# google-deepmind/bsuite

Hardware: NVIDIA H100
Metric: env-steps/sec (higher is better)
Workload: dtype u32 lane state, f64 reward, f32 observation

## Files before the change

bsuite_b200/csrc/bsb_dispatch.cuh:

```cuda
#pragma once
#include <type_traits>
#include <vector>

#include "bsb_env.h"

namespace bsb {

template <class F> struct HostEmit {
  template <class R> static void run(const EnvParams& p, const typename F::Lane& L, R&, float* dst) { F::row(p, L, dst, 1); }
};
template <> struct HostEmit<UmbrellaChain> {
  template <class R> static void run(const EnvParams& p, const UmbrellaChain::Lane& L, R& r, float* dst) { UmbrellaChain::row(p, L, r, dst, 1); }
};
template <> struct HostEmit<DeepSea> {
  template <class R> static void run(const EnvParams& p, const DeepSea::Lane& L, R&, float* dst) {
    for (int e = 0; e < p.obs_numel; ++e) dst[e] = 0.f;
    if (L.hot >= 0) dst[L.hot] = 1.f;
  }
};
template <> struct HostEmit<Catch> {
  template <class R> static void run(const EnvParams& p, const Catch::Lane& L, R&, float* dst) {
    for (int e = 0; e < p.obs_numel; ++e) dst[e] = 0.f;
    dst[L.hot_a] = 1.f; dst[L.hot_b] = 1.f;
  }
};
template <> struct HostEmit<Mnist> {
  template <class R> static void run(const EnvParams& p, const Mnist::Lane& L, R&, float* dst) {
    if (L.image < 0) { for (int e = 0; e < p.obs_numel; ++e) dst[e] = 0.f; return; }
    const int8_t* src = p.images + (int64_t)L.image * p.obs_numel;
    for (int e = 0; e < p.obs_numel; ++e) dst[e] = Mnist::pixel(src[e]);
  }
};

template <class F, int RK, class O, bool kSameStep = false, bool kPacked = false>
void host_run(const EnvParams& p, const LaunchArgs& a) {
  typedef typename RngOf<RK>::type R;
  const int64_t B = p.batch;
  const int K = p.obs_numel;
  O* const obs = reinterpret_cast<O*>(a.obs);
  O* const fin = reinterpret_cast<O*>(a.final_obs);
  std::vector<float> f32(std::is_same<O, float>::value ? 0 : (size_t)K);
  const bool noise = p.wrapper == BSB_WRAP_REWARD_NOISE && a.mode != MODE_INIT;
  const bool track = p.ep != nullptr && a.mode != MODE_INIT;
  const MailFields out = {a.reward, a.reward_f64, a.discount, a.step_type};
  EnvParams setting_p;
  auto render = [&](const EnvParams& lp, const typename F::Lane& L, R& rng, O* dst) {
    if constexpr (std::is_same<O, float>::value) {
      HostEmit<F>::run(lp, L, rng, dst);
    } else {
      HostEmit<F>::run(lp, L, rng, f32.data());
      for (int e = 0; e < K; ++e) dst[e] = obs_cast<O>(f32[(size_t)e]);
    }
  };
  for (int64_t lane = 0; lane < B; ++lane) {
    if constexpr (kPacked) { setting_p = p; pack_lane_params(setting_p, lane); }
    const EnvParams& lp = kPacked ? setting_p : p;
    typename F::Lane L;
    R rng, wrng;
    EpisodeStats ep;
    ActionStream action_stream;
    action_stream.open();
    lane_open<F>(lp, lane, L, rng, wrng, ep, a.mode, noise, track);
    if (a.mode == MODE_INIT) F::ctor_draws(lp, L, rng);
    MergedReset<F, R> merged;
    F::init(p, merged.last);
    merged.done = false;
    for (int64_t t = 0; t < a.T; ++t) {
      const int64_t off = t * B + lane;
      int32_t action = 0;
      if (a.mode == MODE_STEP) {
        action = a.actions ? a.actions[off]
                           : action_stream.sample(a.action_seed, lp.lane_offset + (uint64_t)lane, (uint64_t)(a.step0 + t), p.num_actions);
        if (a.actions_out) a.actions_out[off] = action;
      }
      lane_step<F, R, kSameStep>(lp, lane, L, rng, wrng, ep, action, a.mode, noise, track, a.step0 + t, out, off, &merged);
      if constexpr (kSameStep) { if (merged.done && fin) render(lp, merged.last, merged.rng, fin + off * (int64_t)K); }
      render(lp, L, rng, obs + off * (int64_t)K);
    }
    lane_close<F>(lp, lane, L, rng, wrng, ep, noise, track);
  }
}

struct Geometry { int threads = 0; size_t smem = 0; int64_t n_chunks = 0, grid = 0; int extra_blocks = 0; };

template <class F, class O>
int plan_launch(bsb_env* e, LaunchArgs& a, Geometry& g, bool no_obs = false, int extra_threads = 0) {
  const int K = e->p.obs_numel;
  const bool is_onehot = EmitKind<F>::value == EMIT_ONEHOT;
  const bool is_image = EmitKind<F>::value == EMIT_IMAGE;
  const int64_t B = e->p.batch;
  a.emit_bulk = 1;
  a.group_lanes = 1;
  a.work_counter = nullptr;
  a.work_base = 0;
  const size_t elem = sizeof(O);
  a.stage_rows = ((size_t)2 * 32 * (size_t)K * elem <= 14 * 1024) ? 2 : 1;
  if (a.T == 1 && (EmitKind<F>::value == EMIT_ROWS || EmitKind<F>::value == EMIT_TWOHOT)) a.stage_rows = 1;
  a.cta_extra_elems = 0;
  a.bad_action = e->bad_action_dev;
  int chunk = 32;
  if (is_image)
    while (chunk > 8 && (B + chunk - 1) / chunk < 4 * (int64_t)e->num_sms) chunk >>= 1;
  a.chunk_lanes = chunk;
  g.n_chunks = (B + chunk - 1) / chunk;
  int threads = 64;
  bool persistent = false;
  const size_t tile = (size_t)K * elem;
  if (is_onehot && a.emit_bulk && g.n_chunks >= 4 * (int64_t)e->num_sms && in_compressed_block(a.obs)) a.emit_bulk = 0;
  if (is_onehot && a.emit_bulk) {
    int m = 1;
    while (m < 16 && (size_t)(2 * m) * tile <= 40 * 1024) m <<= 1;
    if (((size_t)m * tile) % 16 != 0 || (size_t)TILE_STAGES * m * tile > 100 * 1024) {
      a.emit_bulk = 0;
    } else {
      a.group_lanes = m; threads = 32; persistent = true;
    }
  }
  if (is_image && a.emit_bulk) {
    int m = 4;
    while (m > 1 && (size_t)m * tile > 28 * 1024) m >>= 1;
    int mz = 8;
    while (mz > 1 && (size_t)mz * tile > 28 * 1024) mz >>= 1;
    if ((K & 15) != 0 || (size_t)m * tile > 64 * 1024) {
      a.emit_bulk = 0;
    } else {
      a.group_lanes = m; a.stage_rows = 1; threads = 128; a.cta_extra_elems = mz * K; persistent = true;
      if (g.n_chunks < 2 * (int64_t)e->num_sms) threads = 64;
    }
  }
  a.use_pdl = (a.mode == MODE_STEP && a.T == 1) ? 1 : 0;
  if (no_obs) { a.emit_bulk = 0; a.stage_rows = 0; a.cta_extra_elems = 0; a.group_lanes = 1; threads = 128; persistent = false; }
  size_t per_warp = smem_elems_per_warp<F, O>(K, a.emit_bulk != 0, a.group_lanes, a.stage_rows) * elem;
  if ((EmitKind<F>::value == EMIT_ROWS || EmitKind<F>::value == EMIT_TWOHOT) && per_warp > 96 * 1024) {
    a.emit_bulk = 0; a.stage_rows = 0; per_warp = 0;
  }
  const size_t cta_extra = (size_t)a.cta_extra_elems * elem;
  size_t smem = per_warp * (size_t)(threads / 32) + cta_extra;
  while (smem > 96 * 1024 && threads > 32) { threads >>= 1; smem = per_warp * (size_t)(threads / 32) + cta_extra; }
  if (smem > 200 * 1024) return fail(BSB_UNSUPPORTED, "observation too large for the staged emitter");
  g.threads = threads;
  g.smem = smem;
  g.extra_blocks = extra_threads > 0 ? (extra_threads / threads > 1 ? extra_threads / threads : 1) : 0;
  g.grid = (g.n_chunks + threads / 32 - 1) / (threads / 32) + g.extra_blocks;
  if (persistent) {
    int64_t per_sm = (int64_t)((227 * 1024) / (smem + 1024));
    per_sm = per_sm < 1 ? 1 : (per_sm > 16 ? 16 : per_sm);
    const int64_t resident = (int64_t)e->num_sms * per_sm;
    if (g.grid > resident) {
      g.grid = resident;
      a.work_counter = a.clock ? a.clock + CLOCK_CHUNK : e->work_counter;
      a.work_base = a.clock ? 0ull : e->work_base;
    }
  }
  return BSB_OK;
}

template <class Kernel, class... Args>
int launch(bsb_env* e, const LaunchArgs& a, const Geometry& g, cudaStream_t stream, Kernel kernel, const Args&... args) {
  if (g.smem > 48 * 1024) BSB_CUDA(cudaFuncSetAttribute(kernel, cudaFuncAttributeMaxDynamicSharedMemorySize, (int)g.smem));
  cudaLaunchConfig_t cfg;
  memset(&cfg, 0, sizeof(cfg));
  cfg.gridDim = dim3((unsigned)g.grid);
  cfg.blockDim = dim3((unsigned)g.threads);
  cfg.dynamicSmemBytes = g.smem;
  cfg.stream = stream;
  cudaLaunchAttribute attr[1];
  if (a.use_pdl) {
    attr[0].id = cudaLaunchAttributeProgrammaticStreamSerialization;
    attr[0].val.programmaticStreamSerializationAllowed = 1;
    cfg.attrs = attr;
    cfg.numAttrs = 1;
  }
  BSB_CUDA(cudaLaunchKernelEx(&cfg, kernel, args...));
  if (a.work_counter && !a.clock) e->work_base += (unsigned long long)g.n_chunks + (unsigned long long)(g.extra_blocks * (g.threads / 32));
  g_launches.fetch_add(1, std::memory_order_relaxed);
  return BSB_OK;
}

template <class F, int RK, bool kNoise, bool kTrack, class O, bool kSameStep = false>
int device_launch(bsb_env* e, LaunchArgs a, cudaStream_t stream) {
  Geometry g;
  const int rc = plan_launch<F, O>(e, a, g);
  return rc != BSB_OK ? rc : launch(e, a, g, stream, transition_kernel<typename KernelTag<F, O, kSameStep>::type, RK, kNoise, kTrack>, e->p, a);
}

template <class F, int RK, bool kNoise, bool kTrack, class O>
int two_phase_launch(bsb_env* e, LaunchArgs a, TwoPhaseArgs h, cudaStream_t stream) {
  if (a.clock) return fail(BSB_INTERNAL, "a host step reached graph-safe mode, which turns the mailbox path off");
  Geometry g;
  const bool obs_only = h.phase == 2;
  const int rc = plan_launch<F, O>(e, a, g, h.phase == 1, obs_only ? 0 : 512);
  if (rc != BSB_OK) return rc;
  h.copiers = g.extra_blocks;
  return launch(e, a, g, stream, two_phase_host_kernel<typename KernelFamily<F, O>::type, RK, kNoise, kTrack>, e->p, a, h);
}

template <class Launch>
int with_flags(const bsb_env* e, const LaunchArgs& a, Launch launch) {
  const bool noise = e->p.wrapper == BSB_WRAP_REWARD_NOISE && a.mode != MODE_INIT;
  const bool track = e->p.ep != nullptr && a.mode != MODE_INIT;
  if (noise) return track ? launch(std::true_type(), std::true_type()) : launch(std::true_type(), std::false_type());
  return track ? launch(std::false_type(), std::true_type()) : launch(std::false_type(), std::false_type());
}

template <class F, class O, bool kSameStep = false>
int run_family_as(bsb_env* e, const LaunchArgs& a, cudaStream_t stream, const TwoPhaseArgs* two_phase) {
  constexpr bool kF32 = std::is_same<O, float>::value && !kSameStep;
  const bool mt = e->p.rng_kind == BSB_RNG_MT19937;
  if (!kF32 && mt) return fail(BSB_INTERNAL, "reduced obs_dtype or same-step auto-reset with MT19937");
  if (kSameStep && two_phase) return fail(BSB_INTERNAL, "a two-phase host step on a same-step handle");
  if (e->device < 0) {
    if constexpr (kF32) { if (mt) { host_run<F, 1, O>(e->p, a); return BSB_OK; } }
    host_run<F, 0, O, kSameStep>(e->p, a);
    return BSB_OK;
  }
// ... 74 lines not shown
```

bsuite_b200/csrc/bsb_kernels.cuh:

```cuda
#pragma once
#include "bsb_families.cuh"

namespace bsb {

struct MailFields {
  float* reward; double* reward_f64; float* discount; int32_t* step_type;
};

struct LaunchArgs {
  const int32_t* actions;
  int32_t* actions_out;
  float* obs;
  float* reward;
  double* reward_f64;
  float* discount;
  int32_t* step_type;
  int64_t T;
  int64_t step0;
  uint64_t action_seed;
  int32_t mode;
  int32_t obs_vec_ok;
  int32_t emit_bulk;
  int32_t use_pdl;
  int32_t group_lanes;
  int32_t final_vec_ok;
  unsigned long long* work_counter;
  unsigned long long work_base;
  unsigned long long* clock;
  int32_t chunk_lanes;
  int32_t stage_rows;
  int32_t cta_extra_elems;
  struct HostMailbox* mailbox;
  struct DeviceMail* mail;
  unsigned long long ticket;
  int32_t timing;
  float* final_obs;
  int32_t* bad_action;
};

struct TwoPhaseArgs {
  int32_t copiers;
  int32_t phase;
  MailFields stage;
};

struct HostMailbox {
  volatile unsigned long long done;     unsigned long long pad[7];
  volatile unsigned long long stamp[8];
};
struct DeviceMail {
  unsigned long long last_exit;
  unsigned long long finished;
  volatile unsigned long long phase1;
  unsigned long long copied;
};

enum { MODE_STEP = 0, MODE_RESET = 1, MODE_INIT = 2 };

template <class Family, class O> struct ObsAs {};
template <class F> struct FamilyOf { typedef F type; };
template <class Family, class O> struct FamilyOf<ObsAs<Family, O> > { typedef Family type; };
template <class F> struct ObsElemOf { typedef float type; };
template <class Family, class O> struct ObsElemOf<ObsAs<Family, O> > { typedef O type; };
template <class Family, class O> struct KernelFamily { typedef ObsAs<Family, O> type; };
template <class Family> struct KernelFamily<Family, float> { typedef Family type; };
template <class O> struct Vec16 { static const int shift = sizeof(O) == 4 ? 2 : sizeof(O) == 2 ? 3 : 4; };
template <class Family, class O> struct SameStep {};
template <class Family, class O> struct FamilyOf<SameStep<Family, O> > { typedef Family type; };
template <class Family, class O> struct ObsElemOf<SameStep<Family, O> > { typedef O type; };
template <class F> struct IsSameStep { static const bool value = false; };
template <class Family, class O> struct IsSameStep<SameStep<Family, O> > { static const bool value = true; };
template <class Family, class O, bool kSameStep> struct KernelTag { typedef typename KernelFamily<Family, O>::type type; };
template <class Family, class O> struct KernelTag<Family, O, true> { typedef SameStep<Family, O> type; };
template <class Family> struct Packed {};
template <class Family> struct FamilyOf<Packed<Family> > { typedef Family type; };
template <class F> struct IsPacked { static const bool value = false; };
template <class Family> struct IsPacked<Packed<Family> > { static const bool value = true; };

template <int RK> struct RngOf;
template <> struct RngOf<0> { typedef LegacyRng<PhiloxSrc> type; };
template <> struct RngOf<1> { typedef LegacyRng<MtSrc> type; };

BSB_HD void rng_open(LegacyRng<PhiloxSrc>& r, const EnvParams& p, int64_t i, bool wrapper) {
  const uint64_t packed = wrapper ? p.wrng_pos[i] : p.rng_pos[i];
  r.src.open(p.seed, p.lane_offset + (uint64_t)i, wrapper ? STREAM_WRAPPER : STREAM_ENV, packed);
  r.g.has = (packed & RNG_HASGAUSS) ? 1 : 0;
  const double* gz = wrapper ? p.wrng_gauss : p.rng_gauss;
  r.g.value = (r.g.has && gz) ? gz[i] : 0.0;
}
BSB_HD void rng_close(const LegacyRng<PhiloxSrc>& r, const EnvParams& p, int64_t i, bool wrapper) {
  const uint64_t packed = r.src.packed() | (r.g.has ? RNG_HASGAUSS : 0ull);
  if (wrapper) p.wrng_pos[i] = packed; else p.rng_pos[i] = packed;
  double* gz = wrapper ? p.wrng_gauss : p.rng_gauss;
  if (gz && r.g.has) gz[i] = r.g.value;
}
BSB_HD void rng_open(LegacyRng<MtSrc>& r, const EnvParams& p, int64_t i, bool wrapper) {
  const int64_t stride = (p.batch > 0) ? p.batch : 1;
  r.src.open((wrapper ? p.wmt_key : p.mt_key) + i, stride, (wrapper ? p.wmt_idx : p.mt_idx)[i]);
  const uint64_t packed = wrapper ? p.wrng_pos[i] : p.rng_pos[i];
  r.g.has = (packed & RNG_HASGAUSS) ? 1 : 0;
  const double* gz = wrapper ? p.wrng_gauss : p.rng_gauss;
  r.g.value = (r.g.has && gz) ? gz[i] : 0.0;
}
BSB_HD void rng_close(const LegacyRng<MtSrc>& r, const EnvParams& p, int64_t i, bool wrapper) {
  (wrapper ? p.wmt_idx : p.mt_idx)[i] = r.src.idx;
// ... 15 lines not shown
    L.nr = (o.step_type == LAST) ? 1u : 0u;
    if (noise) { o.reward = o.reward + p.noise_scale * wrng.randn(); }
    else if (p.wrapper == 2) { o.reward = o.reward * p.reward_scale; }
  }
  return o;
}

template <class F, class R>
BSB_HD void lane_open(const EnvParams& p, int64_t lane, typename F::Lane& L, R& rng, R& wrng, EpisodeStats& ep,
                      int32_t mode, bool noise, bool track, bool state_loaded = false) {
  if (!state_loaded) { if (mode == MODE_INIT) F::init(p, L); else F::load(p, lane, L); }
  if (p.rng_pos) rng_open(rng, p, lane, false);
  if (noise) rng_open(wrng, p, lane, true);
  if (track && !state_loaded) ep.load(p, lane);
}
template <class F, class R>
BSB_HD void lane_close(const EnvParams& p, int64_t lane, const typename F::Lane& L, const R& rng, const R& wrng,
                       const EpisodeStats& ep, bool noise, bool track) {
  F::store(p, lane, L);
  if (p.rng_pos) rng_close(rng, p, lane, false);
  if (noise) rng_close(wrng, p, lane, true);
  if (track) ep.store(p, lane);
}
template <class F> struct ObsDraws { template <class R> static BSB_HD void skip(const EnvParams&, R&) {} };
template <> struct ObsDraws<UmbrellaChain> {
  template <class R> static BSB_HD void skip(const EnvParams& p, R& rng) {
    for (int k0 = 0; k0 < p.n_distractor; k0 += 64) rng.binomial_half_bits((p.n_distractor - k0) < 64 ? (p.n_distractor - k0) : 64);
  }
};
template <class F, class R> struct MergedReset {
  typename F::Lane last;
  R rng;
  bool done;
};

template <class F, class R, bool kSameStep = false>
BSB_HD void lane_step(const EnvParams& p, int64_t lane, typename F::Lane& L, R& rng, R& wrng, EpisodeStats& ep,
                      int32_t action, int32_t mode, bool noise, bool track, int64_t step, const MailFields& out,
                      int64_t off, MergedReset<F, R>* merged = nullptr) {
  bool after_last = L.nr != 0;
  const StepOut o = lane_transition<F, R, R>(p, lane, L, rng, wrng, action, mode, noise);
  if (track) {
    if constexpr (kSameStep) {
      double* restart = p.ep + 5 * p.batch + lane;
      if (*restart != 0.0) {
        *restart = 0.0;
        if (o.step_type == FIRST) after_last = true;
        else { ep.episode_return = 0.0; p.ep[4 * p.batch + lane] = (double)(step - 1); }
      }
    }
    ep.track(p, lane, o, step, after_last);
    if (p.log_rows && o.step_type == LAST && log_row_due(p, lane)) {
      F::store(p, lane, L); ep.store(p, lane);
      log_row_write(p, lane, step + 1);
    }
  }
  if (out.reward) out.reward[off] = (float)o.reward;
  if (out.reward_f64) out.reward_f64[off] = o.reward;
  if (out.discount) out.discount[off] = o.discount;
  if (out.step_type) out.step_type[off] = o.step_type;
  if constexpr (kSameStep) {
    merged->done = o.step_type == LAST;
    if (merged->done) {
      merged->last = L;
      merged->rng = rng;
      ObsDraws<F>::skip(p, rng);
      F::reset(p, lane, L, rng);
      L.nr = 0;
      if (track) p.ep[5 * p.batch + lane] = 1.0;
    }
  }
}

static const int EMIT_ROWS = 0, EMIT_ONEHOT = 1, EMIT_TWOHOT = 2, EMIT_IMAGE = 3;
template <class F> struct ObsFromState { static const bool value = false; };
template <> struct ObsFromState<DeepSea> { static const bool value = true; };
template <> struct ObsFromState<Catch> { static const bool value = true; };
template <class F> struct EmitKind { static const int value = EMIT_ROWS; };
template <> struct EmitKind<DeepSea> { static const int value = EMIT_ONEHOT; };
template <> struct EmitKind<Catch> { static const int value = EMIT_TWOHOT; };
template <> struct EmitKind<Mnist> { static const int value = EMIT_IMAGE; };
static const int ROW_STAGES = 2;
static const int TILE_STAGES = 2;

template <class F> struct BinaryObs {
  static const bool value = EmitKind<F>::value == EMIT_ONEHOT || EmitKind<F>::value == EMIT_TWOHOT;
};

template <class F, class O> inline
#if defined(__CUDACC__)
__host__ __device__
#endif
size_t smem_elems_per_warp(int K, bool emit_bulk, int group_lanes, int row_stages) {
  if (EmitKind<F>::value == EMIT_ROWS || EmitKind<F>::value == EMIT_TWOHOT) return (size_t)row_stages * 32 * (size_t)K;
  if (EmitKind<F>::value == EMIT_ONEHOT && emit_bulk) return (size_t)TILE_STAGES * (size_t)group_lanes * (size_t)K;
  if (EmitKind<F>::value == EMIT_IMAGE)
    return 256 * sizeof(float) / sizeof(O) + (emit_bulk ? (size_t)group_lanes * (size_t)K : 0);
  return 0;
}

#if defined(__CUDACC__)

__device__ __forceinline__ void st_stream(float4* dst, float4 v) { __stcs(dst, v); }
__device__ __forceinline__ void st_stream(float* dst, float v) { __stcs(dst, v); }
__device__ __forceinline__ void st_stream(Bf16* dst, Bf16 v) { __stcs(reinterpret_cast<unsigned short*>(dst), v.bits); }
__device__ __forceinline__ void st_stream(uint8_t* dst, uint8_t v) { __stcs(dst, v); }
template <class O> __device__ __forceinline__ uint32_t one_bits() {
  return sizeof(O) == 2 ? 0x3f80u : 1u;
}
template <class O> struct Quad;
template <> struct Quad<float> { typedef float4 type; static __device__ __forceinline__ float4 of(float4 v) { return v; } };
template <> struct Quad<Bf16> {
  typedef uint2 type;
  static __device__ __forceinline__ uint2 of(float4 v) {
    return make_uint2((uint32_t)f32_to_bf16_bits(v.x) | ((uint32_t)f32_to_bf16_bits(v.y) << 16),
                      (uint32_t)f32_to_bf16_bits(v.z) | ((uint32_t)f32_to_bf16_bits(v.w) << 16));
  }
};
template <> struct Quad<uint8_t> {
  typedef unsigned int type;
  static __device__ __forceinline__ unsigned int of(float4 v) {
    return (uint32_t)f32_to_u8(v.x) | ((uint32_t)f32_to_u8(v.y) << 8) | ((uint32_t)f32_to_u8(v.z) << 16) |
           ((uint32_t)f32_to_u8(v.w) << 24);
  }
};
__device__ __forceinline__ void st_stream(uint2* dst, uint2 v) { __stcs(dst, v); }
__device__ __forceinline__ void st_stream(unsigned int* dst, unsigned int v) { __stcs(dst, v); }

__device__ __forceinline__ void bulk_store_s2g_hint(void* gdst, const void* ssrc, uint32_t bytes, uint64_t policy) {
  const uint32_t s = (uint32_t)__cvta_generic_to_shared(ssrc);
  asm volatile("cp.async.bulk.global.shared::cta.bulk_group.L2::cache_hint [%0], [%1], %2, %3;" ::"l"(gdst), "r"(s), "r"(bytes), "l"(policy) : "memory");
}
__device__ __forceinline__ uint64_t l2_policy_evict_first() {
  uint64_t p; asm("createpolicy.fractional.L2::evict_first.b64 %0, 1.0;" : "=l"(p)); return p;
}
__device__ __forceinline__ void bulk_store_obs(void* gdst, const void* ssrc, uint32_t bytes) {
  bulk_store_s2g_hint(gdst, ssrc, bytes, l2_policy_evict_first());
}
__device__ __forceinline__ void bulk_commit() { asm volatile("cp.async.bulk.commit_group;" ::: "memory"); }
template <int N> __device__ __forceinline__ void bulk_wait_read() { asm volatile("cp.async.bulk.wait_group.read %0;" ::"n"(N) : "memory"); }
__device__ __forceinline__ void fence_proxy_async_smem() { asm volatile("fence.proxy.async.shared::cta;" ::: "memory"); }
__device__ __forceinline__ void pdl_launch_dependents() { asm volatile("griddepcontrol.launch_dependents;" ::: "memory"); }
__device__ __forceinline__ void pdl_wait() { asm volatile("griddepcontrol.wait;" ::: "memory"); }

template <class O>
__device__ __forceinline__ void emit_onehot_vec(O* obs_t, int64_t warp_base, int n_lanes, int K, int hot, bool vec) {
  const int tid = threadIdx.x & 31;
  if (vec && sizeof(O) != 4) {
    constexpr int S = Vec16<O>::shift;
    const int KV = K >> S;
    for (int j = 0; j < n_lanes; ++j) {
      const int h = __shfl_sync(0xffffffffu, hot, j);
      const int hq = h < 0 ? -1 : (h >> S), hb = (h & ((1 << S) - 1)) * (int)sizeof(O);
      const int word = hb >> 2;
      const uint32_t bits = one_bits<O>() << ((hb & 3) * 8);
      uint4* dst = reinterpret_cast<uint4*>(obs_t + (warp_base + j) * (int64_t)K);
#pragma unroll 8
      for (int q = tid; q < KV; q += 32) {
        uint4 v = make_uint4(0u, 0u, 0u, 0u);
        if (q == hq) { if (word == 0) v.x = bits; else if (word == 1) v.y = bits; else if (word == 2) v.z = bits; else v.w = bits; }
        __stcs(dst + q, v);
      }
    }
  } else if (vec) {
    const int K4 = K >> 2;
    for (int j = 0; j < n_lanes; ++j) {
      const int h = __shfl_sync(0xffffffffu, hot, j);
      const int hq = h >> 2, hc = h & 3;
      float4* dst = reinterpret_cast<float4*>(obs_t + (warp_base + j) * (int64_t)K);
#pragma unroll 8
      for (int q = tid; q < K4; q += 32) {
        float4 v = make_float4(0.f, 0.f, 0.f, 0.f);
        if (q == hq) { if (hc == 0) v.x = 1.f; else if (hc == 1) v.y = 1.f; else if (hc == 2) v.z = 1.f; else v.w = 1.f; }
        st_stream(dst + q, v);
      }
    }
  } else {
    for (int j = 0; j < n_lanes; ++j) {
      const int h = __shfl_sync(0xffffffffu, hot, j);
      O* dst = obs_t + (warp_base + j) * (int64_t)K;
      for (int e = tid; e < K; e += 32) st_stream(dst + e, obs_cast<O>(e == h ? 1.f : 0.f));
    }
  }
}

template <class O>
__device__ __forceinline__ void emit_twohot_vec(O* obs_t, int64_t warp_base, int n_lanes, int K, int hot_a, int hot_b, bool vec) {
  const int tid = threadIdx.x & 31;
  const int total = n_lanes * K;
  O* dst = obs_t + warp_base * (int64_t)K;
  constexpr int S = Vec16<O>::shift;
  if (vec && sizeof(O) != 4 && (total & ((1 << S) - 1)) == 0) {
    const int totalV = total >> S;
    for (int q0 = 0; q0 < totalV; q0 += 32) {
      const int q = q0 + tid;
      const int e0 = (q < totalV ? q : 0) << S;
      int j = e0 / K, c = e0 - j * K;
      uint32_t w[4] = {0u, 0u, 0u, 0u};
#pragma unroll
      for (int k = 0; k < (1 << S); ++k) {
        const int jj = j < 32 ? j : 31;
        const int a = __shfl_sync(0xffffffffu, hot_a, jj);
        const int b = __shfl_sync(0xffffffffu, hot_b, jj);
        if (c == a || c == b) w[(k * (int)sizeof(O)) >> 2] |= one_bits<O>() << (((k * (int)sizeof(O)) & 3) * 8);
        if (++c >= K) { c = 0; ++j; }
      }
      if (q < totalV) __stcs(reinterpret_cast<uint4*>(dst) + q, make_uint4(w[0], w[1], w[2], w[3]));
    }
  } else if (vec && (total & ((1 << S) - 1)) == 0) {
    const int total4 = total >> 2;
    for (int q0 = 0; q0 < total4; q0 += 32) {
      const int q = q0 + tid;
      const int e0 = (q < total4 ? q : 0) << 2;
      int j = e0 / K, c = e0 - j * K;
      float v[4];
#pragma unroll
      for (int k = 0; k < 4; ++k) {
        const int jj = j < 32 ? j : 31;
        const int a = __shfl_sync(0xffffffffu, hot_a, jj);
        const int b = __shfl_sync(0xffffffffu, hot_b, jj);
        v[k] = (c == a || c == b) ? 1.f : 0.f;
        if (++c >= K) { c = 0; ++j; }
      }
      if (q < total4) st_stream(reinterpret_cast<float4*>(dst) + q, make_float4(v[0], v[1], v[2], v[3]));
    }
  } else {
    for (int e0 = 0; e0 < total; e0 += 32) {
      const int e = e0 + tid;
      const int ee = e < total ? e : 0;
      const int j = ee / K, c = ee - j * K;
      const int a = __shfl_sync(0xffffffffu, hot_a, j);
      const int b = __shfl_sync(0xffffffffu, hot_b, j);
      if (e < total) st_stream(dst + e, obs_cast<O>((c == a || c == b) ? 1.f : 0.f));
    }
  }
}

template <class O>
__device__ __forceinline__ void emit_image(const EnvParams& p, const float* lut, O* obs_t, int64_t warp_base, int n_lanes, int K, int image, bool vec) {
  const int tid = threadIdx.x & 31;
  constexpr int U = 8;
  for (int j = 0; j < n_lanes; ++j) {
    const int img = __shfl_sync(0xffffffffu, image, j);
    O* dst = obs_t + (warp_base + j) * (int64_t)K;
    const int8_t* src = p.images + (int64_t)(img < 0 ? 0 : img) * K;
    if (vec) {
      const int K4 = K >> 2;
      const uchar4* src4 = reinterpret_cast<const uchar4*>(src);
      typename Quad<O>::type* dst4 = reinterpret_cast<typename Quad<O>::type*>(dst);
      if (img < 0) {
        for (int q = tid; q < K4; q += 32) st_stream(dst4 + q, Quad<O>::of(make_float4(0.f, 0.f, 0.f, 0.f)));
        continue;
      }
      for (int q0 = 0; q0 < K4; q0 += 32 * U) {
        uchar4 c[U];
#pragma unroll
        for (int u = 0; u < U; ++u) {
          const int q = q0 + u * 32 + tid;
          c[u] = make_uchar4(0, 0, 0, 0);
          if (q < K4) c[u] = __ldg(src4 + q);
        }
#pragma unroll
        for (int u = 0; u < U; ++u) {
          const int q = q0 + u * 32 + tid;
          if (q < K4) st_stream(dst4 + q, Quad<O>::of(make_float4(lut[c[u].x], lut[c[u].y], lut[c[u].z], lut[c[u].w])));
        }
      }
    } else {
// ... 65 lines not shown
          }
      }
      fence_proxy_async_smem();
      __syncwarp();
      if (tid == 0) { bulk_store_obs(dst, buf, bytes); bulk_commit(); }
    }
  }
}

template <class O>
__device__ __forceinline__ void flush_rows_vec(const O* stage, O* obs_t, int64_t warp_base, int n_lanes, int K, bool vec) {
  const int tid = threadIdx.x & 31;
  const int total = n_lanes * K;
  O* dst = obs_t + warp_base * (int64_t)K;
  constexpr int S = Vec16<O>::shift;
  if (vec && (total & ((1 << S) - 1)) == 0) {
    const float4* s4 = reinterpret_cast<const float4*>(stage);
    for (int q = tid; q < (total >> S); q += 32) st_stream(reinterpret_cast<float4*>(dst) + q, s4[q]);
  } else {
    for (int e = tid; e < total; e += 32) st_stream(dst + e, stage[e]);
  }
}

template <class F, class R> struct RowRenderer {
  template <class O> static __device__ __forceinline__ void run(const EnvParams& p, const typename F::Lane& L, R&, O* dst) { F::row(p, L, dst, 1); }
};
template <class R> struct RowRenderer<UmbrellaChain, R> {
  template <class O> static __device__ __forceinline__ void run(const EnvParams& p, const UmbrellaChain::Lane& L, R& r, O* dst) { UmbrellaChain::row(p, L, r, dst, 1); }
};
template <class R> struct RowRenderer<DeepSea, R> { template <class O> static __device__ __forceinline__ void run(const EnvParams&, const DeepSea::Lane&, R&, O*) {} };
template <class R> struct RowRenderer<Catch, R> { template <class O> static __device__ __forceinline__ void run(const EnvParams&, const Catch::Lane&, R&, O*) {} };
template <class R> struct RowRenderer<Mnist, R> { template <class O> static __device__ __forceinline__ void run(const EnvParams&, const Mnist::Lane&, R&, O*) {} };

template <class F> struct Descriptor {
  static __device__ __forceinline__ int a(const typename F::Lane&) { return -1; }
  static __device__ __forceinline__ int b(const typename F::Lane&) { return -1; }
};
template <> struct Descriptor<DeepSea> {
  static __device__ __forceinline__ int a(const DeepSea::Lane& L) { return L.hot; }
  static __device__ __forceinline__ int b(const DeepSea::Lane&) { return -1; }
};
template <> struct Descriptor<Catch> {
  static __device__ __forceinline__ int a(const Catch::Lane& L) { return L.hot_a; }
  static __device__ __forceinline__ int b(const Catch::Lane& L) { return L.hot_b; }
};
template <> struct Descriptor<Mnist> {
  static __device__ __forceinline__ int a(const Mnist::Lane& L) { return L.image; }
  static __device__ __forceinline__ int b(const Mnist::Lane&) { return -1; }
};

template <class F> struct MinBlocksPerSM { static const int value = 4; };
template <> struct MinBlocksPerSM<MemoryChain> { static const int value = 6; };
template <> struct MinBlocksPerSM<Bandit> { static const int value = 8; };
template <> struct MinBlocksPerSM<DiscountingChain> { static const int value = 8; };
#define BSB_LAUNCH_MIN_BLOCKS(F) MinBlocksPerSM<typename FamilyOf<F>::type>::value
__device__ __forceinline__ void st_sys_u64(volatile unsigned long long* ptr, unsigned long long v) {
  asm volatile("st.relaxed.sys.global.u64 [%0], %1;" ::"l"(ptr), "l"(v) : "memory");
}
__device__ __forceinline__ unsigned long long global_timer_ns() {
  unsigned long long t; asm volatile("mov.u64 %0, %%globaltimer;" : "=l"(t)); return t;
}
__device__ __forceinline__ void bulk_wait_all() { asm volatile("cp.async.bulk.wait_group 0;" ::: "memory"); }

static const int CLOCK_GROUPS = 32, CLOCK_CHUNK = 16 * CLOCK_GROUPS, CLOCK_TOP = CLOCK_CHUNK + 16,
                 CLOCK_SUB0 = CLOCK_TOP + 16, CLOCK_WORDS = CLOCK_SUB0 + 16 * CLOCK_GROUPS;

template <class O>
struct WarpStage {
  O* stage;
  O* cta_zero;
  unsigned row_mask;
  unsigned emitted = 0;
  int poked_a0 = -1, poked_b0 = -1, poked_a1 = -1, poked_b1 = -1;
  int tile_poked0 = -1, tile_poked1 = -1;
  bool any_bulk = false;
};

template <class F, class O>
__device__ __forceinline__ WarpStage<O> clear_stages(const EnvParams& p, const LaunchArgs& a) {
  extern __shared__ float4 smem_raw[];
  constexpr int kEmit = EmitKind<F>::value;
  const int tid = threadIdx.x & 31, warp = threadIdx.x >> 5, warps_per_cta = blockDim.x >> 5;
  constexpr int S = Vec16<O>::shift;
  const size_t stage_elems = smem_elems_per_warp<F, O>(p.obs_numel, a.emit_bulk != 0, a.group_lanes, a.stage_rows);
  WarpStage<O> ws;
  ws.stage = reinterpret_cast<O*>(smem_raw) + (size_t)warp * stage_elems;
  ws.cta_zero = reinterpret_cast<O*>(smem_raw) + (size_t)warps_per_cta * stage_elems;
  ws.row_mask = a.stage_rows == 2 ? 1u : 0u;
  if (kEmit == EMIT_TWOHOT || (kEmit == EMIT_ONEHOT && a.emit_bulk)) {
    float4* s4 = reinterpret_cast<float4*>(ws.stage);
    const int total4 = (int)(stage_elems >> S);
    for (int q = tid; q < total4; q += 32) s4[q] = make_float4(0.f, 0.f, 0.f, 0.f);
    for (int e = (total4 << S) + tid; e < (int)stage_elems; e += 32) ws.stage[e] = obs_cast<O>(0.f);
    __syncwarp();
  }
  if (kEmit == EMIT_IMAGE) {
    for (int i = tid; i < 256; i += 32) reinterpret_cast<float*>(ws.stage)[i] = Mnist::pixel((int8_t)(uint8_t)i);
    for (int i = threadIdx.x; i < a.cta_extra_elems; i += blockDim.x) ws.cta_zero[i] = obs_cast<O>(0.f);
    fence_proxy_async_smem();
    __syncthreads();
  }
  return ws;
}

__device__ __forceinline__ int64_t fetch_chunk(const LaunchArgs& a, int64_t total_warps) {
  unsigned long long v = 0;
  if ((threadIdx.x & 31) == 0) v = atomicAdd(a.work_counter, 1ull) - a.work_base;
  return total_warps + (int64_t)__shfl_sync(0xffffffffu, v, 0);
}

template <class F, class O>
__device__ __forceinline__ bool chunk_is_bulk(const EnvParams& p, const LaunchArgs& a, bool vec, int n_lanes) {
  constexpr int kEmit = EmitKind<F>::value;
  constexpr int V1 = (1 << Vec16<O>::shift) - 1;
  const int K = p.obs_numel;
  bool bulk = a.emit_bulk && vec;
  if (kEmit == EMIT_ROWS) bulk = bulk && K >= 3 && ((n_lanes * K) & V1) == 0;
  if (kEmit == EMIT_TWOHOT) bulk = bulk && ((n_lanes * K) & V1) == 0;
  if (kEmit == EMIT_ONEHOT) bulk = bulk && ((K & V1) == 0 || ((n_lanes % a.group_lanes) == 0 && ((a.group_lanes * K) & V1) == 0));
  if (kEmit == EMIT_IMAGE) bulk = bulk && (K & 3) == 0;
  return bulk;
}

template <class F, class O, class R>
__device__ __forceinline__ void emit_obs(const EnvParams& p, const LaunchArgs& a, WarpStage<O>& ws, const typename F::Lane& L,
                                         R& rng, O* obs_t, int64_t warp_base, int n_lanes, int64_t lane, bool active,
                                         bool bulk, bool vec) {
  constexpr int kEmit = EmitKind<F>::value;
  constexpr int V1 = (1 << Vec16<O>::shift) - 1;
  const int tid = threadIdx.x & 31;
  const int K = p.obs_numel;
  if (kEmit == EMIT_ONEHOT) {
    const int hot = Descriptor<F>::a(L);
    if (bulk) {
      const int m = a.group_lanes;
      for (int g0 = 0; g0 < n_lanes; g0 += m) {
        const int in_group = (n_lanes - g0) < m ? (n_lanes - g0) : m;
        const int s = (int)(ws.emitted & 1u);
        O* group = ws.stage + (size_t)s * m * K;
        if (tid == 0) bulk_wait_read<TILE_STAGES - 1>();
        __syncwarp();
        if (s == 0) { if (ws.tile_poked0 >= 0) { group[ws.tile_poked0] = obs_cast<O>(0.f); ws.tile_poked0 = -1; } }
        else        { if (ws.tile_poked1 >= 0) { group[ws.tile_poked1] = obs_cast<O>(0.f); ws.tile_poked1 = -1; } }
        __syncwarp();
        if (tid >= g0 && tid < g0 + in_group && hot >= 0) {
          const int cell = (tid - g0) * K + hot;
          group[cell] = obs_cast<O>(1.f);
          if (s == 0) ws.tile_poked0 = cell; else ws.tile_poked1 = cell;
        }
        fence_proxy_async_smem();
        __syncwarp();
        if (tid == 0) {
          O* tile_dst = obs_t + (warp_base + g0) * (int64_t)K;
          const uint32_t tile_bytes = (uint32_t)in_group * (uint32_t)K * (uint32_t)sizeof(O);
          bulk_store_obs(tile_dst, group, tile_bytes);
          bulk_commit();
        }
        ++ws.emitted;
      }
    } else {
      emit_onehot_vec(obs_t, warp_base, n_lanes, K, hot, vec && (K & V1) == 0);
    }
  } else if (kEmit == EMIT_TWOHOT) {
    const int hot_a = Descriptor<F>::a(L), hot_b = Descriptor<F>::b(L);
    if (bulk) {
      const int buf = (int)(ws.emitted & ws.row_mask);
      O* boards = ws.stage + (size_t)buf * 32 * K;
      if (tid == 0) { if (ws.row_mask) bulk_wait_read<1>(); else bulk_wait_read<0>(); }
      __syncwarp();
      O* mine = boards + tid * K;
      const int old_a = buf ? ws.poked_a1 : ws.poked_a0, old_b = buf ? ws.poked_b1 : ws.poked_b0;
      if (old_a >= 0) mine[old_a] = obs_cast<O>(0.f);
      if (old_b >= 0) mine[old_b] = obs_cast<O>(0.f);
      int new_a = -1, new_b = -1;
      if (active) { mine[hot_a] = obs_cast<O>(1.f); mine[hot_b] = obs_cast<O>(1.f); new_a = hot_a; new_b = hot_b; }
      if (buf) { ws.poked_a1 = new_a; ws.poked_b1 = new_b; } else { ws.poked_a0 = new_a; ws.poked_b0 = new_b; }
      fence_proxy_async_smem();
      __syncwarp();
      if (tid == 0) { bulk_store_obs(obs_t + warp_base * (int64_t)K, boards, (uint32_t)n_lanes * (uint32_t)K * (uint32_t)sizeof(O)); bulk_commit(); }
      ++ws.emitted;
    } else {
      emit_twohot_vec(obs_t, warp_base, n_lanes, K, hot_a, hot_b, vec);
    }
  } else if (kEmit == EMIT_IMAGE) {
    const int image = Descriptor<F>::a(L);
    if (bulk) emit_image_bulk(p, ws.stage, ws.cta_zero, obs_t, warp_base, n_lanes, K, active ? image : -1, a.group_lanes,
                              a.cta_extra_elems / K);
    else emit_image(p, reinterpret_cast<const float*>(ws.stage), obs_t, warp_base, n_lanes, K, image, vec && (K & 3) == 0);
  } else if (!a.stage_rows) {
    if (active) RowRenderer<F, R>::run(p, L, rng, obs_t + lane * (int64_t)K);
  } else {
    O* rows = ws.stage + (size_t)(ws.emitted & ws.row_mask) * 32 * K;
    if (bulk) { if (tid == 0) { if (ws.row_mask) bulk_wait_read<1>(); else bulk_wait_read<0>(); } }
    __syncwarp();
    if (active) RowRenderer<F, R>::run(p, L, rng, rows + tid * K);
    if (bulk) {
      fence_proxy_async_smem();
      __syncwarp();
      if (tid == 0) { bulk_store_obs(obs_t + warp_base * (int64_t)K, rows, (uint32_t)n_lanes * (uint32_t)K * (uint32_t)sizeof(O)); bulk_commit(); }
    } else {
      __syncwarp();
      flush_rows_vec(rows, obs_t, warp_base, n_lanes, K, vec);
    }
    ++ws.emitted;
  }
}

template <class F, class O, class R>
__device__ __forceinline__ void emit_final(const EnvParams& p, const LaunchArgs& a, WarpStage<O>& ws, MergedReset<F, R>& m,
                                           O* fin_t, int64_t warp_base, int n_lanes, int64_t lane, bool active, bool vec,
                                           bool obs_bulk) {
  constexpr int kEmit = EmitKind<F>::value;
  const int tid = threadIdx.x & 31;
  const int K = p.obs_numel;
  const unsigned done = __ballot_sync(0xffffffffu, active && m.done);
  if (done == 0u) return;
  const bool bulk = chunk_is_bulk<F, O>(p, a, vec, n_lanes);
  if (done == (n_lanes >= 32 ? 0xffffffffu : ((1u << n_lanes) - 1u)) && (kEmit != EMIT_ROWS || bulk == obs_bulk)) {
    ws.any_bulk = ws.any_bulk || bulk;
    emit_obs<F>(p, a, ws, m.last, m.rng, fin_t, warp_base, n_lanes, lane, active, bulk, vec);
    return;
  }
  if (kEmit == EMIT_ROWS) {
    if (m.done && active) RowRenderer<F, R>::run(p, m.last, m.rng, fin_t + lane * (int64_t)K);
    return;
  }
  const int da = Descriptor<F>::a(m.last), db = Descriptor<F>::b(m.last);
  for (unsigned rest = done; rest != 0u; rest &= rest - 1u) {
    const int j = __ffs(rest) - 1;
    const int a0 = __shfl_sync(0xffffffffu, da, j), b0 = __shfl_sync(0xffffffffu, db, j);
    O* dst = fin_t + (warp_base + j) * (int64_t)K;
    if (kEmit == EMIT_IMAGE) {
      const float* lut = reinterpret_cast<const float*>(ws.stage);
      const int8_t* src = p.images + (int64_t)(a0 < 0 ? 0 : a0) * K;
      for (int e = tid; e < K; e += 32) st_stream(dst + e, obs_cast<O>(a0 >= 0 ? lut[(uint8_t)src[e]] : 0.f));
    } else {
      for (int e = tid; e < K; e += 32) st_stream(dst + e, obs_cast<O>((e == a0 || e == b0) ? 1.f : 0.f));
    }
  }
}

template <class O>
__device__ __forceinline__ void retire_warp(const LaunchArgs& a, const WarpStage<O>& ws, bool drain) {
  if (ws.any_bulk && (threadIdx.x & 31) == 0) { if (drain) bulk_wait_all(); else bulk_wait_read<0>(); }
  if (a.timing && a.mail && threadIdx.x == 0) atomicMax(&a.mail->last_exit, global_timer_ns());
}

__device__ __forceinline__ void signal_done(const LaunchArgs& a) {
  __threadfence_system();
  __syncthreads();
  if (threadIdx.x == 0 && atomicAdd(&a.mail->finished, 1ull) == (unsigned long long)gridDim.x - 1ull) {
    a.mail->finished = 0ull;
    __threadfence_system();
    st_sys_u64(&a.mailbox->done, a.ticket);
  }
}

template <class F, int RK, bool kNoise, bool kTrack>
__global__ void __launch_bounds__(128, BSB_LAUNCH_MIN_BLOCKS(F)) transition_kernel(const EnvParams p, const LaunchArgs a) {
  typedef typename FamilyOf<F>::type Fam;
  typedef typename ObsElemOf<F>::type O;
  typedef typename RngOf<RK>::type R;
  constexpr bool kSameStep = IsSameStep<F>::value;
  constexpr bool kPacked = IsPacked<F>::value;
  const int tid = threadIdx.x & 31, warp = threadIdx.x >> 5, warps_per_cta = blockDim.x >> 5;
  const int64_t B = p.batch;
  const int K = p.obs_numel;
  WarpStage<O> ws = clear_stages<Fam, O>(p, a);
  if (a.use_pdl) { pdl_wait(); pdl_launch_dependents(); }
  int64_t step0 = a.step0;
  if (a.clock) step0 += (int64_t)*reinterpret_cast<volatile unsigned long long*>(a.clock + 16 * (blockIdx.x % CLOCK_GROUPS));
  const MailFields out = {a.reward, a.reward_f64, a.discount, a.step_type};
  const bool vec = a.obs_vec_ok != 0;
  O* const obs = reinterpret_cast<O*>(a.obs);

  const int cl = a.chunk_lanes;
  const int64_t n_chunks = (B + cl - 1) / cl;
  const bool dynamic = a.work_counter != nullptr;
  const int64_t total_warps = (int64_t)gridDim.x * warps_per_cta;
  int64_t cur_chunk = (int64_t)blockIdx.x * warps_per_cta + warp;

  while (cur_chunk < n_chunks) {
    const int64_t warp_base = cur_chunk * cl;
    const int n_lanes = (B - warp_base) < cl ? (int)(B - warp_base) : cl;
    const int64_t lane = warp_base + tid;
    const bool active = tid < n_lanes;
    const bool bulk = chunk_is_bulk<Fam, O>(p, a, vec, n_lanes);
    ws.any_bulk = ws.any_bulk || bulk;
    EnvParams setting_p;
    if constexpr (kPacked) { setting_p = p; if (active) pack_lane_params(setting_p, lane); }
    const EnvParams& lp = kPacked ? setting_p : p;

    typename Fam::Lane L;
    R rng, wrng;
    EpisodeStats ep;
    ActionStream action_stream;
    action_stream.open();
    if (active) lane_open<Fam>(lp, lane, L, rng, wrng, ep, a.mode, kNoise, kTrack);
    else Fam::init(p, L);
    if (a.mode == MODE_INIT && active) Fam::ctor_draws(lp, L, rng);
    MergedReset<Fam, R> merged;
    if constexpr (kSameStep) { Fam::init(p, merged.last); merged.done = false; }

// ... 205 lines not shown
```

Measured before the change: 810.5 million.

## Reuse prior one-hot observation contents and rewrite only differing words

For one-hot environments whose observation buffer sits in a compressed memory block and runs with T==1, the emitter now reads the previous observation tile into shared memory via cp.async, compares it with the new one-hot pattern, and stores only the 16-byte blocks that differ. If a tile differs in more than a couple of words it falls back to blind full writes. This aims to cut global store traffic, since only the old and new hot positions change between steps. The cost is extra global reads, shared-memory staging and warp ballots, and it assumes the buffer still holds the last step's observation.

```diff
diff --git a/bsuite_b200/csrc/bsb_dispatch.cuh b/bsuite_b200/csrc/bsb_dispatch.cuh
--- a/bsuite_b200/csrc/bsb_dispatch.cuh
+++ b/bsuite_b200/csrc/bsb_dispatch.cuh
@@ -106,7 +106,11 @@
   int threads = 64;
   bool persistent = false;
   const size_t tile = (size_t)K * elem;
-  if (is_onehot && a.emit_bulk && g.n_chunks >= 4 * (int64_t)e->num_sms && in_compressed_block(a.obs)) a.emit_bulk = 0;
+  a.emit_reuse = 0;
+  if (is_onehot && a.emit_bulk && g.n_chunks >= 4 * (int64_t)e->num_sms && in_compressed_block(a.obs)) {
+    a.emit_bulk = 0;
+    a.emit_reuse = a.T == 1 ? 1 : 0;
+  }
   if (is_onehot && a.emit_bulk) {
     int m = 1;
     while (m < 16 && (size_t)(2 * m) * tile <= 40 * 1024) m <<= 1;
@@ -129,8 +133,8 @@
     }
   }
   a.use_pdl = (a.mode == MODE_STEP && a.T == 1) ? 1 : 0;
-  if (no_obs) { a.emit_bulk = 0; a.stage_rows = 0; a.cta_extra_elems = 0; a.group_lanes = 1; threads = 128; persistent = false; }
-  size_t per_warp = smem_elems_per_warp<F, O>(K, a.emit_bulk != 0, a.group_lanes, a.stage_rows) * elem;
+  if (no_obs) { a.emit_bulk = 0; a.emit_reuse = 0; a.stage_rows = 0; a.cta_extra_elems = 0; a.group_lanes = 1; threads = 128; persistent = false; }
+  size_t per_warp = smem_elems_per_warp<F, O>(K, a.emit_bulk != 0, a.emit_reuse != 0, a.group_lanes, a.stage_rows) * elem;
   if ((EmitKind<F>::value == EMIT_ROWS || EmitKind<F>::value == EMIT_TWOHOT) && per_warp > 96 * 1024) {
     a.emit_bulk = 0; a.stage_rows = 0; per_warp = 0;
   }
diff --git a/bsuite_b200/csrc/bsb_kernels.cuh b/bsuite_b200/csrc/bsb_kernels.cuh
--- a/bsuite_b200/csrc/bsb_kernels.cuh
+++ b/bsuite_b200/csrc/bsb_kernels.cuh
@@ -21,6 +21,7 @@
   int32_t mode;
   int32_t obs_vec_ok;
   int32_t emit_bulk;
+  int32_t emit_reuse;
   int32_t use_pdl;
   int32_t group_lanes;
   int32_t final_vec_ok;
@@ -202,6 +203,9 @@
 template <> struct EmitKind<Mnist> { static const int value = EMIT_IMAGE; };
 static const int ROW_STAGES = 2;
 static const int TILE_STAGES = 2;
+static const int REUSE_WORDS = 256;
+static const int REUSE_STAGES = 2;
+static const int REUSE_STORE_WORDS = 8;
 
 template <class F> struct BinaryObs {
   static const bool value = EmitKind<F>::value == EMIT_ONEHOT || EmitKind<F>::value == EMIT_TWOHOT;
@@ -211,9 +215,10 @@
 #if defined(__CUDACC__)
 __host__ __device__
 #endif
-size_t smem_elems_per_warp(int K, bool emit_bulk, int group_lanes, int row_stages) {
+size_t smem_elems_per_warp(int K, bool emit_bulk, bool emit_reuse, int group_lanes, int row_stages) {
   if (EmitKind<F>::value == EMIT_ROWS || EmitKind<F>::value == EMIT_TWOHOT) return (size_t)row_stages * 32 * (size_t)K;
   if (EmitKind<F>::value == EMIT_ONEHOT && emit_bulk) return (size_t)TILE_STAGES * (size_t)group_lanes * (size_t)K;
+  if (EmitKind<F>::value == EMIT_ONEHOT && emit_reuse) return (size_t)REUSE_STAGES * REUSE_WORDS * 16 / sizeof(O);
   if (EmitKind<F>::value == EMIT_IMAGE)
     return 256 * sizeof(float) / sizeof(O) + (emit_bulk ? (size_t)group_lanes * (size_t)K : 0);
   return 0;
@@ -304,6 +309,76 @@
   }
 }
 
+__device__ __forceinline__ void cp_async16(void* sdst, const void* gsrc) {
+  asm volatile("cp.async.cg.shared.global [%0], [%1], 16;" ::"r"((uint32_t)__cvta_generic_to_shared(sdst)), "l"(gsrc) : "memory");
+}
+__device__ __forceinline__ void cp_async_commit() { asm volatile("cp.async.commit_group;" ::: "memory"); }
+template <int N> __device__ __forceinline__ void cp_async_wait() { asm volatile("cp.async.wait_group %0;" ::"n"(N) : "memory"); }
+
+template <class O>
+__device__ __forceinline__ void reuse_load(uint4* ring, const O* obs_t, int64_t warp_base, int n_lanes, int K, int s) {
+  const int KV = K >> Vec16<O>::shift;
+  const int passes = (KV + REUSE_WORDS - 1) / REUSE_WORDS;
+  if (s < n_lanes * passes) {
+    const int j = s / passes, q0 = (s - j * passes) * REUSE_WORDS;
+    const uint4* src = reinterpret_cast<const uint4*>(obs_t + (warp_base + j) * (int64_t)K) + q0;
+    uint4* slot = ring + (s % REUSE_STAGES) * REUSE_WORDS;
+    for (int q = threadIdx.x & 31; q < REUSE_WORDS && q0 + q < KV; q += 32) cp_async16(slot + q, src + q);
+  }
+  cp_async_commit();
+}
+template <class O>
+__device__ __forceinline__ uint4 onehot_word(int h, int q) {
+  constexpr int S = Vec16<O>::shift;
+  uint4 v = make_uint4(0u, 0u, 0u, 0u);
+  if (h >= 0 && q == (h >> S)) {
+    const int hb = (h & ((1 << S) - 1)) * (int)sizeof(O), part = hb >> 2;
+    const uint32_t bits = (sizeof(O) == 4 ? 0x3f800000u : one_bits<O>()) << ((hb & 3) * 8);
+    if (part == 0) v.x = bits; else if (part == 1) v.y = bits; else if (part == 2) v.z = bits; else v.w = bits;
+  }
+  return v;
+}
+__device__ __forceinline__ bool bits_differ(uint4 a, uint4 b) { return ((a.x ^ b.x) | (a.y ^ b.y) | (a.z ^ b.z) | (a.w ^ b.w)) != 0u; }
+template <class O>
+__device__ __forceinline__ void emit_onehot_reuse(uint4* ring, O* obs_t, int64_t warp_base, int n_lanes, int K, int hot) {
+  constexpr int S = Vec16<O>::shift;
+  const int tid = threadIdx.x & 31;
+  const int KV = K >> S;
+  const int passes = (KV + REUSE_WORDS - 1) / REUSE_WORDS;
+  const int n = n_lanes * passes;
+  const int h0 = __shfl_sync(0xffffffffu, hot, 0);
+  const uint4* tile0 = reinterpret_cast<const uint4*>(obs_t + warp_base * (int64_t)K);
+  if (tid < KV) cp_async16(ring + tid, tile0 + tid);
+  cp_async_commit();
+  cp_async_wait<0>();
+  bool blind = __popc(__ballot_sync(0xffffffffu, tid < KV && bits_differ(ring[tid], onehot_word<O>(h0, tid)))) > 2;
+  if (!blind) for (int k = 0; k < REUSE_STAGES; ++k) reuse_load(ring, obs_t, warp_base, n_lanes, K, k);
+  for (int s = 0; s < n; ++s) {
+    const int j = s / passes, q0 = (s - j * passes) * REUSE_WORDS;
+    const int h = __shfl_sync(0xffffffffu, hot, j);
+    uint4* dst = reinterpret_cast<uint4*>(obs_t + (warp_base + j) * (int64_t)K) + q0;
+    const uint4* slot = ring + (s % REUSE_STAGES) * REUSE_WORDS;
+    if (!blind) cp_async_wait<REUSE_STAGES - 1>();
+    unsigned differing = 0;
+#pragma unroll 2
+    for (int u = 0; u < REUSE_WORDS / 32 && u * 32 < KV - q0; ++u) {
+      const int q = u * 32 + tid;
+      const bool in = q0 + q < KV;
+      const uint4 v = onehot_word<O>(h, q0 + q);
+      const bool differs = in && (blind || bits_differ(slot[q], v));
+      const unsigned mask = __ballot_sync(0xffffffffu, differs);
+      differing += __popc(mask);
+      const unsigned block = (unsigned)((1ull << REUSE_STORE_WORDS) - 1ull) << (tid & ~(REUSE_STORE_WORDS - 1));
+      if (in && (mask & block) != 0u) __stcs(dst + q, v);
+    }
+    if (!blind) {
+      blind = differing > 2u;
+      if (!blind) reuse_load(ring, obs_t, warp_base, n_lanes, K, s + REUSE_STAGES);
+    }
+  }
+  cp_async_wait<0>();
+}
+
 template <class O>
 __device__ __forceinline__ void emit_twohot_vec(O* obs_t, int64_t warp_base, int n_lanes, int K, int hot_a, int hot_b, bool vec) {
   const int tid = threadIdx.x & 31;
@@ -535,7 +610,7 @@
   constexpr int kEmit = EmitKind<F>::value;
   const int tid = threadIdx.x & 31, warp = threadIdx.x >> 5, warps_per_cta = blockDim.x >> 5;
   constexpr int S = Vec16<O>::shift;
-  const size_t stage_elems = smem_elems_per_warp<F, O>(p.obs_numel, a.emit_bulk != 0, a.group_lanes, a.stage_rows);
+  const size_t stage_elems = smem_elems_per_warp<F, O>(p.obs_numel, a.emit_bulk != 0, a.emit_reuse != 0, a.group_lanes, a.stage_rows);
   WarpStage<O> ws;
   ws.stage = reinterpret_cast<O*>(smem_raw) + (size_t)warp * stage_elems;
   ws.cta_zero = reinterpret_cast<O*>(smem_raw) + (size_t)warps_per_cta * stage_elems;
@@ -574,11 +649,15 @@
   if (kEmit == EMIT_IMAGE) bulk = bulk && (K & 3) == 0;
   return bulk;
 }
+template <class O>
+__device__ __forceinline__ bool reuse_chunk(const LaunchArgs& a, bool vec, int K) {
+  return a.emit_reuse && vec && (K & ((1 << Vec16<O>::shift) - 1)) == 0;
+}
 
 template <class F, class O, class R>
 __device__ __forceinline__ void emit_obs(const EnvParams& p, const LaunchArgs& a, WarpStage<O>& ws, const typename F::Lane& L,
                                          R& rng, O* obs_t, int64_t warp_base, int n_lanes, int64_t lane, bool active,
-                                         bool bulk, bool vec) {
+                                         bool bulk, bool vec, bool reuse = true) {
   constexpr int kEmit = EmitKind<F>::value;
   constexpr int V1 = (1 << Vec16<O>::shift) - 1;
   const int tid = threadIdx.x & 31;
@@ -611,6 +690,8 @@
         }
         ++ws.emitted;
       }
+    } else if (reuse && reuse_chunk<O>(a, vec, K)) {
+      emit_onehot_reuse(reinterpret_cast<uint4*>(ws.stage), obs_t, warp_base, n_lanes, K, hot);
     } else {
       emit_onehot_vec(obs_t, warp_base, n_lanes, K, hot, vec && (K & V1) == 0);
     }
@@ -671,7 +752,7 @@
   const bool bulk = chunk_is_bulk<F, O>(p, a, vec, n_lanes);
   if (done == (n_lanes >= 32 ? 0xffffffffu : ((1u << n_lanes) - 1u)) && (kEmit != EMIT_ROWS || bulk == obs_bulk)) {
     ws.any_bulk = ws.any_bulk || bulk;
-    emit_obs<F>(p, a, ws, m.last, m.rng, fin_t, warp_base, n_lanes, lane, active, bulk, vec);
+    emit_obs<F>(p, a, ws, m.last, m.rng, fin_t, warp_base, n_lanes, lane, active, bulk, vec, false);
     return;
   }
   if (kEmit == EMIT_ROWS) {
```

Result: faster. 916.1 million (median of 6 runs) (+13.0%).
